# thilinarmtb/lsbench

Hardware: AMD Instinct MI355X
Metric: cg_solves_per_sec (higher is better)
Workload: dtype f64

## Files before the change

include/lsbench_hip.h:

```cpp
#ifndef LSBENCH_HIP_H
#define LSBENCH_HIP_H

#include "lsbench.h"
#include <stddef.h>

#ifdef __cplusplus
extern "C" {
#endif


struct lsbench {
  char *matrix;
  lsbench_solver_t solver;
  lsbench_ordering_t ordering;
  lsbench_precision_t precision;
  unsigned verbose, trials;
};

struct csr {
  unsigned nrows, base;
  unsigned *offs, *cols;
  double *vals;
};

// ... 247 lines not shown
void lsb_plan_exchange(int me, int nall, const unsigned *hull,
                       struct lsb_xfer *recv, int *nrecv,
                       struct lsb_xfer *send, int *nsend);
struct csr *lsbench_matrix_synth(const char *spec, unsigned r0, unsigned r1,
                                 unsigned *n_global);


typedef struct lsb_hip_solver lsb_hip_solver;

lsb_hip_solver *lsb_hip_solver_create(const struct csr *A,
                                      const struct lsb_hip_opts *o);
lsb_hip_solver *lsb_hip_solver_create_dist(const struct csr *A_rows,
                                           unsigned row_begin,
                                           unsigned n_global,
                                           const struct lsb_hip_opts *o);
void lsb_hip_solver_destroy(lsb_hip_solver *s);

int lsb_hip_solver_solve(lsb_hip_solver *s, const double *b, double *x,
                         struct lsb_hip_result *res);
int lsb_hip_solver_solve_dev(lsb_hip_solver *s, const double *d_b, double *d_x,
                             struct lsb_hip_result *res);
int lsb_hip_solver_spmv_dev(lsb_hip_solver *s, const double *d_x, double *d_y);
int lsb_hip_solver_spmv_inner_dev(lsb_hip_solver *s, const double *d_x, double *d_y, double *d_dot);
int lsb_hip_solver_precond_dev(lsb_hip_solver *s, const double *d_r, double *d_z);
int lsb_hip_solver_amg_info(lsb_hip_solver *s, unsigned *levels, unsigned *tail_levels);
int lsb_hip_solver_cheb_interval(const lsb_hip_solver *s, double *lmin, double *lmax);
int lsb_hip_solver_time_spmv(lsb_hip_solver *s, int warm, int reps,
                             double *ms_avg);
int lsb_hip_solver_jacobi_sweep_dev(lsb_hip_solver *s, double w,
                                    const double *d_b, double *d_x);

unsigned lsb_hip_solver_nrows_local(const lsb_hip_solver *s);
int lsb_hip_solver_padded(const lsb_hip_solver *s);
unsigned lsb_hip_solver_nrows_global(const lsb_hip_solver *s);
unsigned long long lsb_hip_solver_nnz_local(const lsb_hip_solver *s);
unsigned lsb_hip_solver_nblocks(const lsb_hip_solver *s);
int lsb_hip_solver_spmv_variant(const lsb_hip_solver *s);
unsigned lsb_hip_solver_spmv_flags(const lsb_hip_solver *s);
unsigned lsb_hip_solver_spmv_grid(const lsb_hip_solver *s);
unsigned lsb_hip_solver_spmv_period(const lsb_hip_solver *s);
unsigned long long lsb_hip_solver_spmv_col_slices(const lsb_hip_solver *s);
void lsb_hip_solver_sell_value_slots(const lsb_hip_solver *s, unsigned *kept, unsigned *total);
int lsb_hip_solver_overlaps(const lsb_hip_solver *s);
int lsb_hip_solver_comm(const lsb_hip_solver *s, double *p2p_us, double *rccl_us);
void lsb_hip_solver_comm_plan(const lsb_hip_solver *s, unsigned long long plan[8]);
int lsb_hip_solver_overlap(const lsb_hip_solver *s, double us[2]);
unsigned long long lsb_hip_solver_spmv_layout_bytes(const lsb_hip_solver *s);
unsigned long long lsb_hip_solver_iteration_bytes(const lsb_hip_solver *s);
int lsb_hip_solver_single_reduction(const lsb_hip_solver *s);
int lsb_hip_solver_fused_p(const lsb_hip_solver *s);
int lsb_hip_solver_blas1_nt(const lsb_hip_solver *s);
void *lsb_hip_stream(void);


#define LSB_HIP_UNIQUE_ID_BYTES 128
int lsb_hip_comm_get_unique_id(void *id128);
int lsb_hip_comm_init_rank(const void *id128, int nranks, int rank);
int lsb_hip_comm_destroy(void);
int lsb_hip_comm_rank(void);
int lsb_hip_comm_size(void);
int lsb_hip_comm_count(void);
int lsb_hip_comm_allreduce_sum_dev(double *d_buf, int count);
int lsb_hip_comm_barrier(void);


#define LSB_SPMV_FLAG_PREFETCH 1u
// ... 36 lines not shown
```

lsbench_amd/_lib.py:

```python
import ctypes as C
import os
import subprocess

_CSRC = os.path.join(os.path.dirname(os.path.abspath(__file__)), "csrc")
LIB_PATH = os.path.join(_CSRC, "liblsbench_hip.so")
CORE_PATH = os.path.join(_CSRC, "liblsbench_core.so")
CORE_SYMBOLS = ("lsbench_matrix_read", "lsbench_matrix_print", "lsbench_matrix_free", "lsbench_init",
                "lsbench_get_matrix_name", "lsbench_bench", "lsbench_finalize")

UNIQUE_ID_BYTES = 128

SOLVER_HIP = 6
OP_CHOLMOD_UPPER, OP_RAW = 0, 1
PRECOND_JACOBI, PRECOND_NONE, PRECOND_L1JACOBI, PRECOND_CHEBYSHEV, PRECOND_BLOCKJACOBI, PRECOND_FSAI = 0, 1, 2, 3, 4, 5
PRECOND_AMG = 6
KRYLOV_PCG, KRYLOV_GMRES, KRYLOV_PCG1, KRYLOV_AUTO, KRYLOV_BICGSTAB = 0, 1, 2, 3, 4
SPMV_AUTO, SPMV_ADAPTIVE, SPMV_SUBWAVE, SPMV_SCALAR, SPMV_PANEL, SPMV_SELL, SPMV_BINNED, SPMV_TWOPHASE = 0, 1, 2, 3, 4, 5, 6, 7
SELL_ROWS = 128
BIN_CHUNK = 2048
PB_COLS, PB_ROWS = 8192, 2048
SPMV_FLAG_PREFETCH, SPMV_FLAG_NT, SPMV_FLAG_C16, SPMV_FLAG_TMPL, SPMV_FLAG_DEFER, SPMV_FLAG_COL = 1, 2, 4, 64, 128, 256
STATUS_RUNNING, STATUS_CONVERGED, STATUS_BREAKDOWN, STATUS_MAXIT = 0, 1, 2, 3
STATUS_COMM = 4
COMM_AUTO, COMM_RCCL, COMM_P2P = 0, 1, 2
# ... 157 lines not shown
    "lsb_sell_vc_free": (None, [C.POINTER(SellVc)]),
    "lsb_csr_fsai_pattern": (C.POINTER(FsaiPattern), [_csrp, _i, _u]),
    "lsb_fsai_pattern_free": (None, [C.POINTER(FsaiPattern)]),
    "lsb_amg_setup": (C.POINTER(AmgHier), [_csrp, _d, _u, _u]),
    "lsb_amg_aggregate": (C.POINTER(C.c_int), [_csrp, _d, C.POINTER(_u)]),
    "lsb_amg_free": (None, [C.POINTER(AmgHier)]),
    "lsb_sell16_templates": (C.POINTER(SellTmpls), [C.POINTER(Sell), C.POINTER(SellVc)]),
    "lsb_sell_tmpls_free": (None, [C.POINTER(SellTmpls)]),
    "lsb_tmpl_check": (_i, [C.POINTER(Sell), C.POINTER(SellVc), C.POINTER(SellTmpls), _u, _u, _u, _i,
                            C.c_char_p, C.c_size_t]),
    "lsb_sell_tmpl_columns": (C.POINTER(TmplCols), [C.POINTER(SellTmpls), _u, _u]),
    "lsb_sell_tmpl_columns_range": (C.POINTER(TmplCols), [C.POINTER(SellTmpls), _u, _u, _u, _u]),
    "lsb_tmpl_cols_free": (None, [C.POINTER(TmplCols)]),
    "lsb_tmpl_cols_check": (_i, [C.POINTER(SellTmpls), C.POINTER(TmplCols), C.c_char_p, C.c_size_t]),
    "lsb_csr_mean_scatter": (_d, [_csrp, _u]),
    "lsb_csr_col_hull": (None, [_csrp, C.POINTER(_u), C.POINTER(_u)]),
    "lsb_plan_exchange": (None, [_i, _i, C.POINTER(_u), C.POINTER(Xfer), C.POINTER(_i),
                                 C.POINTER(Xfer), C.POINTER(_i)]),
    "lsbench_matrix_synth": (_csrp, [C.c_char_p, _u, _u, C.POINTER(_u)]),
    "lsb_hip_solver_create": (_vp, [_csrp, C.POINTER(Opts)]),
    "lsb_hip_solver_create_dist": (_vp, [_csrp, _u, _u, C.POINTER(Opts)]),
    "lsb_hip_solver_destroy": (None, [_vp]),
    "lsb_hip_solver_solve": (_i, [_vp, _vp, _vp, C.POINTER(Result)]),
    "lsb_hip_solver_solve_dev": (_i, [_vp, _vp, _vp, C.POINTER(Result)]),
    "lsb_hip_solver_spmv_dev": (_i, [_vp, _vp, _vp]),
    "lsb_hip_solver_spmv_inner_dev": (_i, [_vp, _vp, _vp, _vp]),
    "lsb_hip_solver_precond_dev": (_i, [_vp, _vp, _vp]),
    "lsb_hip_solver_amg_info": (_i, [_vp, C.POINTER(_u), C.POINTER(_u)]),
    "lsb_hip_solver_cheb_interval": (_i, [_vp, C.POINTER(_d), C.POINTER(_d)]),
    "lsb_hip_solver_time_spmv": (_i, [_vp, _i, _i, C.POINTER(_d)]),
    "lsb_hip_solver_jacobi_sweep_dev": (_i, [_vp, _d, _vp, _vp]),
    "lsb_hip_solver_nrows_local": (_u, [_vp]),
    "lsb_hip_solver_padded": (_i, [_vp]),
    "lsb_csr_pad_lines": (_csrp, [_csrp, _u, C.POINTER(_u), C.POINTER(_u), C.POINTER(C.POINTER(C.c_int))]),
    "lsb_hip_solver_nrows_global": (_u, [_vp]),
    "lsb_hip_solver_nnz_local": (C.c_ulonglong, [_vp]),
    "lsb_hip_solver_nblocks": (_u, [_vp]),
    "lsb_hip_solver_spmv_variant": (_i, [_vp]),
    "lsb_hip_solver_spmv_flags": (_u, [_vp]),
    "lsb_hip_solver_spmv_grid": (_u, [_vp]),
    "lsb_hip_solver_spmv_period": (_u, [_vp]),
    "lsb_hip_solver_spmv_col_slices": (C.c_ulonglong, [_vp]),
    "lsb_hip_solver_sell_value_slots": (None, [_vp, C.POINTER(C.c_uint), C.POINTER(C.c_uint)]),
    "lsb_hip_solver_overlaps": (_i, [_vp]),
    "lsb_hip_solver_overlap": (_i, [_vp, C.POINTER(C.c_double)]),
    "lsb_hip_solver_comm_plan": (None, [_vp, C.POINTER(C.c_ulonglong)]),
    "lsb_hip_solver_spmv_layout_bytes": (C.c_ulonglong, [_vp]),
    "lsb_hip_solver_fused_p": (_i, [_vp]),
    "lsb_hip_solver_iteration_bytes": (C.c_ulonglong, [_vp]),
    "lsb_hip_solver_single_reduction": (_i, [_vp]),
    "lsb_hip_solver_blas1_nt": (_i, [_vp]),
    "lsb_hip_solver_comm": (_i, [_vp, C.POINTER(C.c_double), C.POINTER(C.c_double)]),
    "lsb_hip_stream": (_vp, []),
    "lsb_hip_comm_get_unique_id": (_i, [_vp]),
    "lsb_hip_comm_init_rank": (_i, [_vp, _i, _i]),
    "lsb_hip_comm_destroy": (_i, []),
    "lsb_hip_comm_rank": (_i, []),
    "lsb_hip_comm_size": (_i, []),
    "lsb_hip_comm_count": (_i, []),
    "hip_cdna4_set_option": (_i, [C.c_char_p, C.c_char_p]),
    "hip_cdna4_matrix_synth": (_csrp, [C.c_char_p]),
    "lsb_hip_comm_allreduce_sum_dev": (_i, [_vp, _i]),
    "lsb_hip_comm_barrier": (_i, []),
    "lsb_hip_spmv_csr_f64": (_i, [_i, _u, _vp, _vp, _vp, _vp, _vp, _u, _u, _u, _vp, _vp,
                                  _vp, _vp, _vp, _vp]),
    "lsb_hip_partials_capacity": (_u, []),
# ... 62 lines not shown
```

lsbench_amd/api.py:

```python
import ctypes as C

import numpy as np

from . import _lib as L


def _ptr(a):
    if a is None:
        return None
    if hasattr(a, "data_ptr"):
        return a.data_ptr()
    if isinstance(a, np.ndarray):
        return a.ctypes.data
    return int(a)


class Matrix:

    def __init__(self, handle):
        if not handle:
            raise L.LsbenchHipError("NULL struct csr")
        self._h = handle

    @classmethod
# ... 252 lines not shown
        return lo.value, hi.value

    def time_spmv(self, warm=5, reps=50):
        ms = C.c_double()
        L.check(L.load().lsb_hip_solver_time_spmv(self._h, warm, reps, C.byref(ms)),
                "time_spmv")
        return ms.value

    def jacobi_sweep_dev(self, w, d_b, d_x):
        L.check(L.load().lsb_hip_solver_jacobi_sweep_dev(self._h, w, _ptr(d_b), _ptr(d_x)),
                "jacobi_sweep_dev")

    @property
    def nblocks(self):
        return L.load().lsb_hip_solver_nblocks(self._h)

    @property
    def spmv_variant(self):
        return L.load().lsb_hip_solver_spmv_variant(self._h)

    @property
    def spmv_flags(self):
        return L.load().lsb_hip_solver_spmv_flags(self._h)

    @property
    def spmv_grid(self):
        return L.load().lsb_hip_solver_spmv_grid(self._h)

    @property
    def padded(self):
        return int(L.load().lsb_hip_solver_padded(self._h))

    @property
    def spmv_col_slices(self):
        return int(L.load().lsb_hip_solver_spmv_col_slices(self._h))

    @property
    def spmv_period(self):
        return L.load().lsb_hip_solver_spmv_period(self._h)

    @property
    def sell_value_slots(self):
        import ctypes as C
        k, t = C.c_uint(0), C.c_uint(0)
        L.load().lsb_hip_solver_sell_value_slots(self._h, C.byref(k), C.byref(t))
        return int(k.value), int(t.value)

    @property
    def spmv_layout_bytes(self):
        return int(L.load().lsb_hip_solver_spmv_layout_bytes(self._h))

    @property
    def iteration_bytes(self):
        return int(L.load().lsb_hip_solver_iteration_bytes(self._h))

    @property
    def single_reduction(self):
        return bool(L.load().lsb_hip_solver_single_reduction(self._h))

    @property
    def fused_p(self):
        return int(L.load().lsb_hip_solver_fused_p(self._h))

    @property
    def blas1_nt(self):
        return int(L.load().lsb_hip_solver_blas1_nt(self._h))
# ... 34 lines not shown
```

lsbench_amd/csrc/hip_kernels.hip:

```cpp
#include "hip_kcommon.h"

__device__ __forceinline__ void spmv_publish(double *__restrict__ partials, double dot,
                                             double *sred, const lsb_ar_tail &tail) {
  if (!partials)
    return;
  double d[1] = {dot};
  wg_sum<1>(d, sred);
  if (tail.counter)
    ar_tail(partials, d[0], tail);
  else if (threadIdx.x == 0)
    partials[blockIdx.x] = d[0];
}

enum { SP_PREFETCH = 1, SP_NT = 2 };

template <int FLAGS, class T>
__device__ __forceinline__ T stream_load(const T *p) {
  if (FLAGS & SP_NT)
    return __builtin_nontemporal_load(p);
  return *p;
}

#define LSB_ISSUE_BLOCK(kk)                                                    \
  do {                                                                         \
// ... 1189 lines not shown
        colp_compute<NF, true, XUPD>(c0, m0, pm, p0, pp, down, C, vm0, vm1, vp0, vp1, beta, alpha, alpha2, dc, lane, res, dot);
        COLP_STORE(res, lrow, false, true);
        pm = p0, p0 = pp, c0 = c1, m0 = m1, m1 = m2;
        gu += D, lrow += Du;
      }
      colp_issue_c<NF, false, NT>(c1, C, r, pold, x, pnew, gu + D, D, n, lane);
      colp_compute<NF, true, XUPD>(c0, m0, pm, p0, pp, down, C, vm0, vm1, vp0, vp1, beta, alpha, alpha2, dc, lane, res, dot);
      COLP_STORE(res, lrow, false, true);
      pm = p0, p0 = pp, c0 = c1, m0 = m1;
      gu += D, lrow += Du;
      colp_compute<NF, false, XUPD>(c0, m0, pm, p0, pp, down, C, vm0, vm1, vp0, vp1, beta, alpha, alpha2, dc, lane, res, dot);
      COLP_STORE(res, lrow, false, false);
    } else {
      for (unsigned k = 0; k < K; k++)
        colp_single(s + k * period, n, lane, sptr, sbase, vals, vconst, r, pold, pnew, x, nullptr, beta, alpha, alpha2,
                    XUPD, dc, dot);
    }
  }
  if (partials) {
    double d[1] = {dot};
    wg_sum<1>(d, sred);
    if (threadIdx.x == 0)
      partials[blockIdx.x] = d[0];
  }
}
#undef COLP_STORE
#undef COLP_ST

template <int NF>
__global__ __launch_bounds__(WG, 5) void k_pcg_col_r(
    const unsigned *__restrict__ plan, unsigned period, unsigned n, const unsigned *__restrict__ sptr,
    const unsigned long long *__restrict__ mask, const lsb_sell_tmpl *__restrict__ td, const int *__restrict__ sbase,
    const double *__restrict__ vals, const double *__restrict__ vconst, const double *__restrict__ p,
    double *__restrict__ r, double dc, lsb_pcg_state *__restrict__ st, int parity, int pbuf, int xtwo,
    const double *__restrict__ pq_parts, unsigned npq, double *__restrict__ partials2) {
  static_assert(NF >= 1 && NF <= 2, "one or two far slots per side");
  __shared__ double sred[8];
  const unsigned tid = threadIdx.x, lane = tid & 63u, wave = tid >> 6;
  const unsigned gx = gridDim.x / NXCD, xcd = blockIdx.x % NXCD, slot = blockIdx.x / NXCD;
  const int stopped = st->status, pad = st->pad;
  const double rz = st->rz[parity];
  const unsigned i0 = plan[xcd], i1 = plan[xcd + 1];
  double pqv[1];
  wg_sum_partials<1>(pq_parts, npq, pqv, sred);
  if (stopped)
    return;
  if (pad) {
    if (blockIdx.x == 0 && threadIdx.x == 0)
      st->status = LSB_STATUS_MAXIT;
    return;
  }
  const double pq = pqv[0];
  if (!(pq != 0.0) || !isfinite(pq)) {
    if (blockIdx.x == 0 && threadIdx.x == 0)
      st->status = LSB_STATUS_BREAKDOWN;
    return;
  }
  const double alpha = rz / pq;
  if (blockIdx.x == 0 && threadIdx.x == 0) {
    st->pq = pq, st->alpha[1] = st->alpha[0], st->alpha[0] = alpha, st->xpend = (xtwo ? 3 : 1) + pbuf;
  }
  const u4v *__restrict__ items = (const u4v *)(plan + LSB_COL_HEAD);
  const unsigned dofs = plan[LSB_TMPL_COL_DOWN];
  const unsigned P = period * LSB_SELL_ROWS;
  double acc[2] = {0.0, 0.0}, nodot = 0.0;
#define COLR_FINISH(A0, A1, RV, LROW)                                                          \
  do {                                                                                         \
    sell_d2v rn_;                                                                              \
    rn_.x = (RV).x - alpha * (A0), rn_.y = (RV).y - alpha * (A1);                              \
    *(sell_d2v *)(r + (LROW) + 2 * lane) = rn_;                                                \
    acc[0] += rn_.x * (dc * rn_.x);                                                            \
    acc[0] += rn_.y * (dc * rn_.y);                                                            \
    acc[1] += rn_.x * rn_.x;                                                                   \
    acc[1] += rn_.y * rn_.y;                                                                   \
  } while (0)
  for (unsigned g = slot; i0 + 4 * g < i1; g += gx) {
    const unsigned it = __builtin_amdgcn_readfirstlane(i0 + 4 * g + wave);
    if (it >= i1)
      continue;
    const u4v rec = items[it];
    const unsigned s = __builtin_amdgcn_readfirstlane(rec.x);
    const unsigned K = __builtin_amdgcn_readfirstlane(rec.y) & ~LSB_TMPL_COL_LOCKSTEP;
    if (K >= 3) {
      const unsigned t = __builtin_amdgcn_readfirstlane(rec.z), mb = __builtin_amdgcn_readfirstlane(rec.w);
      const lsb_sell_tmpl *T = td + t;
      col_tmpl<NF> C;
      C.bc = T->base[NF + 1];
      C.k0 = T->cst[0], C.kc = T->cst[NF + 1], C.kL = T->cst[2 * NF + 2];
#pragma unroll
      for (int k = 0; k < NF - 1; k++) {
        C.bl[k] = T->base[1 + k], C.bh[k] = T->base[NF + 3 + k];
        C.kl[k] = T->cst[1 + k], C.kh[k] = T->cst[NF + 3 + k];
      }
      const int side_k[2] = {T->kidx[NF], T->kidx[NF + 2]}, side_kd[2] = {T->kind[NF], T->kind[NF + 2]};
      const bool down = col_walks_down(plan, dofs, it);
      const unsigned s0 = down ? s + (K - 1) * period : s;
      const long long D = down ? -(long long)P : (long long)P;
      const unsigned Du = (unsigned)D;
      long long gu = (long long)s0 * LSB_SELL_ROWS;
      unsigned lrow = s0 * LSB_SELL_ROWS;
      col_ops<NF> cur, nxt;
      sell_d2u cb = *(const sell_d2u *)(p + (gu + C.bc - D) + 2 * lane);
      sell_d2u c0 = *(const sell_d2u *)(p + (gu + C.bc) + 2 * lane);
      sell_d2u ca, cn;
      col_issue<NF, 2>(cur, ca, C, p, r, gu, lrow, D, n, lane, true);
      unsigned long long mk[2][2] = {{0ull, 0ull}, {0ull, 0ull}};
#pragma unroll
      for (int side = 0; side < 2; side++)
        if (side_k[side] >= 0 && side_kd[side] == 2) {
// ... 411 lines not shown
  if (period < NXCD || !plan)
    errx(EXIT_FAILURE, "lsb_k_spmv_tmpl_col: no column plan (period %u)", period);
  const sell_launch L = sell_prologue("lsb_k_spmv_tmpl_col", true, c, nitem, n, grid_cap, 0, period, partials,
                                      npartials, tail_in);
  const int f32 = (flags & LSB_SP_F32) != 0;
  const int dot = !partials || !xdot ? 0 : (xdot == x + row_begin && centre0) ? 1 : 2;
  static decltype(&k_spmv_tmpl_col<1, 0>) const kern[2][3] = {
      {k_spmv_tmpl_col<1, 0>, k_spmv_tmpl_col<1, 1>, k_spmv_tmpl_col<1, 2>},
      {k_spmv_tmpl_col<2, 0>, k_spmv_tmpl_col<2, 1>, k_spmv_tmpl_col<2, 2>}};
  kern[c->tmpl.nfar - 1][dot]<<<L.g, WG, 0, (hipStream_t)stream>>>(
      plan, L.period, n, row_begin, xlen, c->sptr, c->tmpl.mask, c->tmpl.td, c->sbase, c->vals, f32, c->vconst, x, y,
      xdot, partials, st, L.tail);
}

void lsb_k_pcg_col_px(unsigned grid_cap, unsigned period, const unsigned *plan, unsigned nitem, unsigned n,
                      const struct lsb_sell16_dev *c, const double *r, const double *pold, double *pnew, double *x,
                      int xupd, double dc, double *partials, unsigned *npartials, struct lsb_pcg_state *st, int parity,
                      const double *parts2, unsigned nparts2, void *stream) {
  if (period < NXCD || !plan || pold == pnew)
    errx(EXIT_FAILURE, "lsb_k_pcg_col_px: no column plan (period %u) or one direction buffer", period);
  const unsigned nfar = c->tmpl.nfar;
  const sell_launch L = sell_prologue("lsb_k_pcg_col_px", true, c, nitem, n, grid_cap, LSB_TMPL_COL_GRID(nfar), period,
                                      partials, npartials, NULL);
  static decltype(&k_pcg_col_px<1, 3, false>) const kern[2][2] = {
      {k_pcg_col_px<1, 3, false>, k_pcg_col_px<1, 3, true>},
      {k_pcg_col_px<2, 3, false>, k_pcg_col_px<2, 3, true>}};
  kern[nfar - 1][xupd != 0]<<<L.g, WG, 0, (hipStream_t)stream>>>(
      plan, L.period, n, c->sptr, c->tmpl.mask, c->tmpl.td, c->sbase, c->vals, c->vconst, r, pold, pnew, x, dc,
      partials, st, parity, parts2, nparts2);
}

void lsb_k_pcg_col_r(unsigned grid_cap, unsigned period, const unsigned *plan, unsigned nitem, unsigned n,
                     const struct lsb_sell16_dev *c, const double *p, double *r, double dc, struct lsb_pcg_state *st,
                     int parity, int pbuf, int xtwo, const double *pq_parts, unsigned npq, double *partials2,
                     unsigned *npartials, void *stream) {
  if (period < NXCD || !plan)
    errx(EXIT_FAILURE, "lsb_k_pcg_col_r: no column plan (period %u)", period);
  const sell_launch L = sell_prologue("lsb_k_pcg_col_r", true, c, nitem, n, grid_cap, LSB_TMPL_COL_GRID(1), period,
                                      partials2, npartials, NULL);
  const auto kern = c->tmpl.nfar == 1 ? k_pcg_col_r<1> : k_pcg_col_r<2>;
  kern<<<L.g, WG, 0, (hipStream_t)stream>>>(plan, L.period, n, c->sptr, c->tmpl.mask, c->tmpl.td, c->sbase, c->vals,
                                            c->vconst, p, r, dc, st, parity, pbuf, xtwo, pq_parts, npq, partials2);
}

}
```

lsbench_amd/csrc/hip_pcg.c:

```c
#define _GNU_SOURCE
#include "hip_solver.h"

#define DINV(s) ((s)->dinv_uniform ? NULL : (s)->d_dinv), (s)->dinv_const

enum pcg_form pcg_choose_form(const lsb_hip_solver *sv) {
  const struct shard *s = &sv->sh[0];
  const struct lsb_hip_opts *o = &sv->o;
  if (o->krylov == LSB_KRYLOV_GMRES || o->krylov == LSB_KRYLOV_BICGSTAB)
    return PCG_NONE;
  if (o->precond == LSB_PRECOND_FSAI && !sv->multi && !s->mixed && s->variant == LSB_SPMV_SUBWAVE &&
      s->fs_g.variant == LSB_SPMV_SUBWAVE && s->fs_gt.variant == LSB_SPMV_SUBWAVE && o->sample_spmv <= 0 &&
      o->krylov != LSB_KRYLOV_PCG1 && !getenv("LSBENCH_HIP_NO_FSAI_FUSE"))
    return PCG_FSAI3;
  if (generic_precond(sv))
    return PCG_GENERIC;
  if (o->krylov == LSB_KRYLOV_PCG1 || (o->krylov == LSB_KRYLOV_AUTO && sv->multi))
    return PCG_CG1;
  if (sv->multi || s->mixed || getenv("LSBENCH_HIP_NO_FUSE_P"))
    return PCG_CLASSIC;
  if (s->sell_form == SELL_COL && s->dinv_uniform && s->c16.tmpl.nfar >= 1 && s->c16.tmpl.nfar <= 2 &&
      s->row_begin == 0 && s->n == s->n_glob && o->precond == LSB_PRECOND_JACOBI && !getenv("LSBENCH_HIP_NO_FUSE_PX"))
    return PCG_COL;
  return s->variant == LSB_SPMV_SUBWAVE && o->sample_spmv <= 0 ? PCG_SUBWAVE : PCG_CLASSIC;
}
// ... 153 lines not shown
    sv->pcur = 0;
    spmv_shard(s, buf[0], s->d_q, buf[0], s->d_parts_pq, &s->npq, s->d_st);
  } else {
    lsb_k_spmv_subwave_p(s->n, s->csr.offs, s->csr.cols, s->csr.vals, s->lanes, s->d_r, DINV(s),
                         buf[sv->pcur], buf[sv->pcur ^ 1], s->d_q, s->d_parts_pq, &s->npq, s->d_st,
                         parity ^ 1, s->d_parts2, s->np2, g_stream);
    sv->pcur ^= 1;
  }
  lsb_k_pcg_update_xr(s->n, buf[sv->pcur], s->d_q, DINV(s), d_x, s->d_r, s->d_st, parity,
                      s->d_parts_pq, s->npq, s->d_parts2, &s->np2, sv->nt_mask, g_stream);
  if (pos & 2)
    lsb_k_pcg_update_p(s->n, s->d_r, DINV(s), buf[sv->pcur], buf[0], s->d_st, parity, s->d_parts2,
                       s->np2, sv->nt_mask, g_stream);
}

static void col_enqueue_iter(lsb_hip_solver *sv, double *d_x, int parity, int pos, int sample) {
  struct shard *s = &sv->sh[0];
  double *buf[2] = {s->d_pfull, s->d_p1};
  if (sample >= 0)
    sv->samp_skip[sample] = (pos & 1) != 0;
  if (pos & 1) {
    sv->pcur = 0;
    spmv_shard(s, buf[0], s->d_q, buf[0], s->d_parts_pq, &s->npq, s->d_st);
  } else {
    sample_open(sv, sample);
    lsb_k_pcg_col_px(s->sp_grid, s->col.period, s->col.plan, s->col.items, s->n, &s->c16, s->d_r, buf[sv->pcur],
                     buf[sv->pcur ^ 1], d_x,  parity == 0,
                     s->dinv_const, s->d_parts_pq, &s->npq, s->d_st, parity ^ 1, s->d_parts2, s->np2, g_stream);
    sample_close(sv, sample);
    sv->pcur ^= 1;
  }
  lsb_k_pcg_col_r(s->sp_grid, s->col.period, s->col.plan, s->col.items, s->n, &s->c16, buf[sv->pcur], s->d_r,
                  s->dinv_const, s->d_st,
                  parity, sv->pcur,  parity != 0, s->d_parts_pq, s->npq,
                  s->d_parts2, &s->np2, g_stream);
  if (pos & 2) {
    lsb_k_pcg_xfix(s->n, buf[0], buf[1], d_x, s->d_st, g_stream);
    lsb_k_pcg_update_p(s->n, s->d_r, DINV(s), buf[sv->pcur], buf[0], s->d_st, parity, s->d_parts2, s->np2,
                       sv->nt_mask, g_stream);
  }
}

static void cg1_enqueue_init(lsb_hip_solver *sv, const double *d_b, double *d_x) {
  sv->ar_fold = can_fold_allreduce(sv), sv->ar_pending = 0, sv->fold_next = 0;
  for (int i = 0; i < sv->nshard; i++) {
    struct shard *s = &sv->sh[i];
    const size_t o = s->row_begin - sv->row_first, bytes = (size_t)s->n * sizeof(double);
    if (sv->cg1_implicit)
      lsb_k_pcg_init(s->n, d_b + o, DINV(s), d_x + o, s->d_pfull + s->row_begin, s->d_r,
                     s->d_parts2, &s->np2, g_stream);
    else
      lsb_k_pcg_init(s->n, d_b + o, DINV(s), d_x + o, s->d_r, s->d_pfull + s->row_begin,
                     s->d_parts2, &s->np2, g_stream);
    LSB_CHK_HIP(hipMemsetAsync(s->d_p1, 0, bytes, g_stream));
    LSB_CHK_HIP(hipMemsetAsync(s->d_s1, 0, bytes, g_stream));
  }
  init_state(sv);
  spmv_pq(sv, -1);
}

static void cg1_enqueue_iter(lsb_hip_solver *sv, double *d_x, int parity, int sample) {
  for (int i = 0; i < sv->nshard; i++) {
    struct shard *s = &sv->sh[i];
    const size_t o = s->row_begin - sv->row_first;
    double *gr_in = s->d_parts2 + (size_t)parity * 2 * LSB_MAX_PARTIALS;
    double *gr_out = s->d_parts2 + (size_t)(parity ^ 1) * 2 * LSB_MAX_PARTIALS;
    unsigned np2 = 0;
    struct lsb_ar_collect col;
// ... 591 lines not shown
```

lsbench_amd/csrc/hip_solver.c:

```c
#define _GNU_SOURCE
#include "hip_solver.h"
#define NXCD_HOST 8u

unsigned pow2_ceil(unsigned v) {
  unsigned p = 1;
  while (p < v)
    p <<= 1;
  return p;
}

void choose_spmv(struct shard *s, const struct lsb_hip_opts *o) {
  const unsigned mean = s->n ? (unsigned)((s->nnz + s->n - 1) / s->n) : 1;
  int v = o->spmv_variant;
  if (v == LSB_SPMV_AUTO)
    v = s->nnz <= 500000ull ? LSB_SPMV_SUBWAVE : LSB_SPMV_ADAPTIVE;
  if (v == LSB_SPMV_PANEL && !s->panel.n)
    v = LSB_SPMV_ADAPTIVE;
  if (v == LSB_SPMV_BINNED && !s->bins.n)
    v = LSB_SPMV_ADAPTIVE;
  if (v == LSB_SPMV_TWOPHASE && !s->tp.bins)
    v = LSB_SPMV_ADAPTIVE;
  if (v == LSB_SPMV_SELL && !s->sell.sptr)
    v = LSB_SPMV_ADAPTIVE;
  s->variant = v;
// ... 381 lines not shown
  }
  if (s->nnz == 0)
    lo = hi = row_begin;
  s->col_lo = lo, s->col_hi = hi;
  if ((unsigned long long)s->nnz > 0x7FFFFFFFull || n_glob > 0x7FFFFFFFu)
    errx(EXIT_FAILURE, "shard too large for int32 device indices");
  s->mixed = o->precision == LSB_PREC_MIXED, s->exact32 = 1;
  struct csr G = {n, 0, (unsigned *)offs, (unsigned *)cols, (double *)(S->vals + j0)};
  csr_build(s, &G);
  const char *e = getenv("LSBENCH_HIP_PANEL_COLS");
  const unsigned width = e ? (unsigned)strtoul(e, NULL, 10) : 524288u;
  const int scattered = s->nnz > 4000000ull && (double)(hi - lo) * 8.0 > 16.0e6 &&
                        lsb_csr_mean_scatter(&G, row_begin) > 1.0e6;
  if (width && o->spmv_variant == LSB_SPMV_PANEL)
    panel_build(&s->panel, &G, width);
  if (width && (o->spmv_variant == LSB_SPMV_BINNED || (o->spmv_variant == LSB_SPMV_AUTO && scattered)))
    bins_build(&s->bins, &G, width);
  if (o->spmv_variant == LSB_SPMV_TWOPHASE || (o->spmv_variant == LSB_SPMV_AUTO && scattered))
    tp_build(&s->tp, &G, n_glob);
  sell_build(s, &G, o);
  if (s->sell.sptr) {
    struct lsb_sell_vc *V = NULL;
    struct lsb_sell *H = c16_build(s, &G, &V);
    struct lsb_sell_tmpls *TT = V ? tmpl_build(s, H, V) : NULL;
    if (TT)
      col_build(s, H, V, TT);
    LSB_CHK_HIP(hipStreamSynchronize(g_stream));
    lsb_sell_tmpls_free(TT), lsb_sell_vc_free(V), lsb_sell_free(H);
  }
  precond_shard_blocks(s, offs, cols, S->vals + j0, o);
  LSB_CHK_HIP(hipStreamSynchronize(g_stream));
  free(offs), free(cols);

  {
    size_t cnt = 3 * (size_t)n + n_glob;
    if (n_glob > n || o->nvirt > 1 || o->krylov == LSB_KRYLOV_PCG1)
      cnt += 2 * (size_t)n;
    if (o->precond == LSB_PRECOND_CHEBYSHEV)
      cnt += 2 * (size_t)n_glob + (size_t)n;
    else if (o->precond == LSB_PRECOND_BLOCKJACOBI)
      cnt += (size_t)n;
    else if (o->precond == LSB_PRECOND_FSAI)
      cnt += 4 * (size_t)n;
    else if (o->precond == LSB_PRECOND_AMG)
      cnt += 3 * (size_t)n;
    if (o->krylov == LSB_KRYLOV_BICGSTAB)
      cnt += 3 * (size_t)n + n_glob;
    if (o->krylov != LSB_KRYLOV_GMRES && !getenv("LSBENCH_HIP_NO_SLAB") && (size_t)n * sizeof(double) <= ((size_t)160 << 20)) {
      s->slab_cap = cnt * sizeof(double) + 16 * 256;
      if (hipMalloc((void **)&s->d_slab, s->slab_cap) != hipSuccess)
        s->d_slab = NULL, s->slab_cap = 0, (void)hipGetLastError();
    }
  }
  s->d_r = shard_vec(s, n);
  s->d_q = shard_vec(s, n);
  s->d_pfull = shard_vec(s, n_glob);
  s->d_dinv = shard_vec(s, n);
  LSB_CHK_HIP(hipMemsetAsync(s->d_pfull, 0, (size_t)n_glob * sizeof(double), g_stream));
  s->d_parts_pq = (double *)lsb_hip_malloc(3 * LSB_MAX_PARTIALS * sizeof(double));
  s->d_parts2 = (double *)lsb_hip_malloc(4 * LSB_MAX_PARTIALS * sizeof(double));
  s->d_st = (struct lsb_pcg_state *)lsb_hip_malloc(sizeof(struct lsb_pcg_state));
  LSB_CHK_HIP(hipMemsetAsync(s->d_st, 0, sizeof(struct lsb_pcg_state), g_stream));
  s->d_st_aux = (struct lsb_pcg_state *)lsb_hip_malloc(sizeof(struct lsb_pcg_state));
  LSB_CHK_HIP(hipMemsetAsync(s->d_st_aux, 0, sizeof(struct lsb_pcg_state), g_stream));
  choose_spmv(s, o);

  if (o->precond == LSB_PRECOND_JACOBI || o->precond == LSB_PRECOND_L1JACOBI ||
      o->precond == LSB_PRECOND_CHEBYSHEV) {
    int *d_nz = (int *)lsb_hip_malloc(sizeof(int)), nz = 0;
    LSB_CHK_HIP(hipMemsetAsync(d_nz, 0, sizeof(int), g_stream));
    if (o->precond == LSB_PRECOND_L1JACOBI)
      lsb_k_l1_setup(n, s->csr.offs, s->csr.vals, s->d_dinv, d_nz, g_stream);
    else
      lsb_k_jacobi_setup(n, row_begin, s->csr.offs, s->csr.cols, s->csr.vals, s->d_dinv, d_nz,
                         g_stream);
    LSB_CHK_HIP(hipMemcpyAsync(&nz, d_nz, sizeof(int), hipMemcpyDeviceToHost, g_stream));
    LSB_CHK_HIP(hipStreamSynchronize(g_stream));
    lsb_hip_free(d_nz);
    if (nz)
      errx(EXIT_FAILURE, "hip_cdna4: %d rows have no non-zero %s; "
                         "Jacobi preconditioning needs one (cf. the stored-diagonal "
                         "assumption of src/cholmod-impl.h:13)", nz,
           o->precond == LSB_PRECOND_L1JACOBI ? "entry" : "diagonal entry");
  } else {
    double *ones = (double *)malloc((size_t)(n ? n : 1) * sizeof(double));
    for (unsigned i = 0; i < n; i++)
      ones[i] = 1.0;
    LSB_CHK_HIP(hipMemcpy(s->d_dinv, ones, (size_t)n * sizeof(double), hipMemcpyHostToDevice));
    free(ones);
  }
  if (n && !getenv("LSBENCH_HIP_NO_UNIFORM_DINV")) {
// ... 105 lines not shown
  bicgstab_check_precond(&o);
  if (o.precision == LSB_PREC_MIXED && o.precond == LSB_PRECOND_AMG) {
    warnx("hip_cdna4: --precond amg runs in fp64");
    o.precision = LSB_PREC_FP64;
  }
  struct csr *S = o.op_mode == LSB_OP_CHOLMOD_UPPER ? lsb_csr_symmetrize_upper(A)
                                                    : lsb_csr_copy_base0(A);
  const unsigned n_user = S->nrows;
  int *padmap = NULL;
  {
    const char *e = getenv("LSBENCH_HIP_PAD_LINES");
    const int want = e ? atoi(e) : (S->nrows >= 1000000u ? 1 : 0);
    if (want && !o.reorder) {
      unsigned nx = 0, nxp = 0;
      struct csr *Sp = lsb_csr_pad_lines(S, LSB_SELL_ROWS, &nx, &nxp, &padmap);
      if (Sp) {
        if (o.verbose)
          fprintf(stderr, "hip_cdna4: grid lines of %u rows padded to %u (%u -> %u rows)\n", nx, nxp, S->nrows,
                  Sp->nrows);
        lsb_csr_free(S);
        S = Sp;
      }
    }
  }
  int P = o.nvirt > 1 ? o.nvirt : 1;
  if ((unsigned)P > S->nrows / 2)
    P = 1;
  lsb_hip_solver *sv = solver_alloc(P, &o);
  sv->n_user = n_user;
  if (padmap) {
    sv->d_perm = (int *)dev_upload(padmap, (size_t)S->nrows * sizeof(int));
    LSB_CHK_HIP(hipStreamSynchronize(g_stream));
    free(padmap);
    sv->d_bp = (double *)lsb_hip_malloc((size_t)S->nrows * sizeof(double));
    sv->d_xp = (double *)lsb_hip_malloc((size_t)S->nrows * sizeof(double));
    sv->padded = 1;
  }
  if (o.reorder) {
    unsigned *perm = (unsigned *)malloc((size_t)S->nrows * sizeof(unsigned));
    if (!perm || lsb_csr_rcm(S, perm))
      errx(EXIT_FAILURE, "hip_cdna4: out of memory computing the RCM ordering");
    struct csr *Sp = lsb_csr_permute_sym(S, perm);
    if (o.verbose)
      fprintf(stderr, "hip_cdna4: RCM bandwidth %u -> %u\n", lsb_csr_bandwidth(S),
              lsb_csr_bandwidth(Sp));
    lsb_csr_free(S);
    S = Sp;
    sv->d_perm = (int *)dev_upload(perm, (size_t)S->nrows * sizeof(int));
    LSB_CHK_HIP(hipStreamSynchronize(g_stream));
    free(perm);
    sv->d_bp = (double *)lsb_hip_malloc((size_t)S->nrows * sizeof(double));
    sv->d_xp = (double *)lsb_hip_malloc((size_t)S->nrows * sizeof(double));
  }
  sv->n_glob = sv->n_here = S->nrows, sv->row_first = 0;
  sv->dist = 0, sv->multi = P > 1;
  unsigned *bounds = lsb_calloc(unsigned, (size_t)P + 1);
  lsb_csr_partition_rows(S, (unsigned)P, bounds);
  unsigned *hull = lsb_calloc(unsigned, 4 * (size_t)P);
  for (int q = 0; q < P; q++) {
    shard_upload(&sv->sh[q], S, bounds[q], bounds[q + 1], 0, bounds[q], S->nrows, &o);
    hull[4 * q] = bounds[q], hull[4 * q + 1] = bounds[q + 1] - bounds[q];
    hull[4 * q + 2] = sv->sh[q].col_lo, hull[4 * q + 3] = sv->sh[q].col_hi;
  }
  for (int q = 0; q < P; q++) {
    plan_exchange(&sv->sh[q], q, P, hull);
    for (int k = 0; k < sv->sh[q].nrecv; k++)
      if (sv->sh[q].recv[k].count > sv->agree_halo)
        sv->agree_halo = (unsigned)sv->sh[q].recv[k].count;
  }
  free(hull), free(bounds);
  lsb_csr_free(S);
  solver_finish_setup(sv);
  return sv;
}

lsb_hip_solver *lsb_hip_solver_create_dist(const struct csr *A_rows,
                                           unsigned row_begin,
                                           unsigned n_global,
                                           const struct lsb_hip_opts *o_in) {
  if (!lsb_initialized || !A_rows)
    return NULL;
  struct lsb_hip_opts o;
  if (o_in)
    o = *o_in;
  else
    lsb_hip_get_opts(&o);
  if (o.precision == LSB_PREC_MIXED &&
      (o.krylov == LSB_KRYLOV_GMRES || o.krylov == LSB_KRYLOV_BICGSTAB || o.precond == LSB_PRECOND_AMG))
    o.precision = LSB_PREC_FP64;
  bicgstab_check_precond(&o);
  const int P = lsb_hip_comm_size(), me = lsb_hip_comm_rank();
  lsb_hip_solver *sv = solver_alloc(1, &o);
  sv->n_glob = n_global, sv->n_here = sv->n_user = A_rows->nrows, sv->row_first = row_begin;
  const char *alone = getenv("LSBENCH_HIP_DIST_ALONE");
  sv->dist = sv->multi = P > 1 || (alone && atoi(alone) > 0);
// ... 30 lines not shown
    sv->sh[0].nsend = 1, sv->sh[0].send[0].peer = -1;
    sv->sh[0].send[0].offset = row_begin, sv->sh[0].send[0].count = A_rows->nrows;
    sv->sh[0].nrecv = 0;
  }
  free(hull);
  {
    unsigned h = 0, *allh = lsb_calloc(unsigned, (size_t)P);
    for (int k = 0; k < sv->sh[0].nrecv; k++)
      if (sv->sh[0].recv[k].count > h)
        h = (unsigned)sv->sh[0].recv[k].count;
    lsb_hip_comm_allgather_u32(&h, 1, allh);
    for (int q = 0; q < P; q++)
      if (allh[q] > sv->agree_halo)
        sv->agree_halo = allh[q];
    free(allh);
  }
  solver_finish_setup(sv);
  return sv;
}

void lsb_hip_solver_destroy(lsb_hip_solver *sv) {
  if (!sv)
    return;
  LSB_CHK_HIP(hipStreamSynchronize(g_stream));
  drop_graphs(sv);
  if (sv->p2p) {
    if (sv->dist)
      lsb_hip_comm_barrier();
    for (int i = 0; i < sv->nshard; i++)
      lsb_p2p_destroy(sv->p2p[i]);
    free(sv->p2p);
  }
  bicgstab_free(sv);
  for (int i = 0; i < sv->nshard; i++)
    shard_free(&sv->sh[i]);
  if (sv->have_events) {
    for (int i = 0; i < 4 * MAX_SAMPLES; i++)
      LSB_CHK_HIP(hipEventDestroy(sv->ev[i]));
    LSB_CHK_HIP(hipEventDestroy(sv->ev_t0));
    LSB_CHK_HIP(hipEventDestroy(sv->ev_t1));
    LSB_CHK_HIP(hipEventDestroy(sv->ev_poll[0]));
    LSB_CHK_HIP(hipEventDestroy(sv->ev_poll[1]));
    LSB_CHK_HIP(hipEventDestroy(sv->ev_vec));
    LSB_CHK_HIP(hipEventDestroy(sv->ev_halo));
  }
  lsb_hip_free(sv->d_scal_all), lsb_hip_free(sv->d_tmp);
  lsb_hip_free(sv->d_vr), lsb_hip_free(sv->d_ve);
  lsb_hip_free(sv->ps.d_wgrow), lsb_hip_free(sv->ps.d_ug), lsb_hip_free(sv->ps.d_shared);
  lsb_hip_free(sv->d_perm), lsb_hip_free(sv->d_bp), lsb_hip_free(sv->d_xp);
  for (int i = 0; sv->gm && i < sv->nshard; i++) {
    lsb_hip_free(sv->gm[i].V), lsb_hip_free(sv->gm[i].parts);
    lsb_hip_free(sv->gm[i].ax), lsb_hip_free(sv->gm[i].st);
  }
  free(sv->gm);
  lsb_hip_free(sv->gm_red);
  if (sv->gm_hst)
    LSB_CHK_HIP(hipHostFree(sv->gm_hst));
  LSB_CHK_HIP(hipHostFree(sv->h_st));
  free(sv->sh), free(sv);
}

unsigned lsb_hip_solver_nrows_local(const lsb_hip_solver *s) { return s->n_user; }
int lsb_hip_solver_padded(const lsb_hip_solver *s) { return s->padded ? (int)(s->n_here - s->n_user) : 0; }
unsigned lsb_hip_solver_nrows_global(const lsb_hip_solver *s) { return s->n_glob; }
unsigned long long lsb_hip_solver_nnz_local(const lsb_hip_solver *s) {
  unsigned long long z = 0;
  for (int i = 0; i < s->nshard; i++)
    z += s->sh[i].nnz;
  return z;
}
unsigned lsb_hip_solver_nblocks(const lsb_hip_solver *s) { return s->sh[0].csr.nblk; }
int lsb_hip_solver_spmv_variant(const lsb_hip_solver *s) { return s->sh[0].variant; }
unsigned lsb_hip_solver_spmv_flags(const lsb_hip_solver *s) { return s->sh[0].sp_flags; }
unsigned lsb_hip_solver_spmv_grid(const lsb_hip_solver *s) { return s->sh[0].sp_grid; }
unsigned lsb_hip_solver_spmv_period(const lsb_hip_solver *s) { return s->sh[0].sp_period; }
unsigned long long lsb_hip_solver_spmv_col_slices(const lsb_hip_solver *s) { return s->sh[0].col.slices; }
void lsb_hip_solver_sell_value_slots(const lsb_hip_solver *s, unsigned *kept, unsigned *total) {
  const struct shard *h = &s->sh[0];
  const int on = h->sell_form >= SELL_16;
  if (kept)
    *kept = on ? h->c16.vslots : 0;
  if (total)
    *total = on ? h->c16.slots : 0;
}
void lsb_hip_solver_comm_plan(const lsb_hip_solver *s, unsigned long long plan[8]) {
  const struct shard *h = &s->sh[0];
  memset(plan, 0, 8 * sizeof plan[0]);
  plan[0] = (unsigned long long)lsb_hip_comm_count();
  plan[6] = (unsigned long long)s->nshard;
  if (!s->multi)
    return;
  plan[5] = h->nsend == 1 && h->send[0].peer == -1;
  if (plan[5]) {
    const unsigned long long P = s->dist ? (unsigned long long)lsb_hip_comm_size() : (unsigned long long)s->nshard;
    plan[1] = plan[2] = P - 1;
// ... 383 lines not shown
```

lsbench_amd/csrc/hip_solver.h:

```cpp
#ifndef HIP_SOLVER_H
#define HIP_SOLVER_H

#define __HIP_PLATFORM_AMD__ 1
#include <hip/hip_runtime_api.h>
#include <math.h>
#include <string.h>
#include <strings.h>
#include <time.h>

#include "lsb_impl.h"

#define LSB_INTERNAL __attribute__((visibility("hidden")))

extern LSB_INTERNAL int lsb_initialized;
extern LSB_INTERNAL __thread hipStream_t g_stream;
extern LSB_INTERNAL __thread struct lsb_hip_result g_last;
LSB_INTERNAL hipStream_t comm_stream(void);
LSB_INTERNAL void rank_thread_attach(int device);
LSB_INTERNAL void rank_thread_detach(void);
LSB_INTERNAL int bench_multi(double *x, struct csr *A, const double *r, const struct lsbench *cb,
                             const struct lsb_hip_opts *o, int ngpus);

#define SCAL_STRIDE 8
#define MAX_SAMPLES 64
#define LSB_NGRAPH 4

struct halo_split {
  unsigned first, last;
  int ok;
};
enum { SELL_NONE, SELL_32, SELL_16, SELL_TMPL, SELL_COL };
enum pcg_form {
  PCG_NONE,
  PCG_CLASSIC,
  PCG_SUBWAVE,
  PCG_COL,
  PCG_CG1,
  PCG_GENERIC,
  PCG_FSAI3,
};

struct shard {
  char *d_slab;
  size_t slab_cap, slab_used;
  unsigned row_begin, n;
  unsigned long long nnz;
  unsigned n_glob;
  unsigned col_lo, col_hi;
  int variant, sell_form;
  unsigned lanes;
  unsigned sp_flags, sp_grid, sp_period;
  int mixed, exact32;
  struct shard_csr {
    int *offs, *cols, *rowblk;
    unsigned char *blklanes;
    double *vals;
    float *vals32;
    unsigned nblk;
    struct halo_split split;
  } csr;
  struct shard_panel {
    unsigned n;
    unsigned *blk;
    int *offs, *cols, *rowmap, *rowblk;
    unsigned char *blklanes;
    double *vals;
  } panel;
  struct shard_bins {
    unsigned n, cap;
    unsigned *chunk_h;
    unsigned *chunk, *rows, *cols;
    double *vals;
  } bins;
  struct shard_tp {
    unsigned items, bins, col_lo, xlen, cols, rows;
    unsigned *item, *binptr, *first, *delta;
    unsigned long long *mask;
// ... 197 lines not shown
```

lsbench_amd/csrc/lsb_impl.h:

```cpp
#ifndef LSB_IMPL_H
#define LSB_IMPL_H

#include "lsbench_hip.h"
#include <err.h>
#include <stdint.h>
#include <stdio.h>
#include <stdlib.h>

#ifdef __cplusplus
extern "C" {
#endif

#define lsb_calloc(T, n) ((T *)calloc((size_t)(n) > 0 ? (size_t)(n) : 1, sizeof(T)))

struct lsb_pcg_state {
  double rz[2];
  double bb;
  double thresh2;
  double rr;
  double pq;
  double alpha[2];
  int iters;
  int status;
  int maxit;
// ... 66 lines not shown
                     const int *sbase, const double *vals, const double *vconst, unsigned ulen,
                     const double *x, double *y, const double *xdot, double *partials,
                     unsigned *npartials,
                     const struct lsb_pcg_state *st, const struct lsb_ar_tail *tail,
                     const struct lsb_cheb_epi *epi, void *stream);
#define LSB_SP_TMPL 64u
#define LSB_SP_DEFER 128u
struct lsb_sell16_dev {
  unsigned *sptr;
  short *codes;
  int *sbase;
  double *vals;
  double *vconst;
  unsigned vslots, slots, ulen;
  unsigned long long bytes;
  struct lsb_tmpl_dev {
    unsigned *srec;
    unsigned long long *mask;
    struct lsb_sell_tmpl *td;
    unsigned nfar;
    unsigned long long bytes;
  } tmpl;
};
void lsb_k_spmv_tmpl(unsigned flags, unsigned grid_cap, unsigned period, const struct lsb_sell16_dev *c, unsigned s0,
                     unsigned ns, unsigned n, unsigned row_begin, unsigned xlen, const double *x, double *y,
                     const double *xdot, double *partials, unsigned *npartials, const struct lsb_pcg_state *st,
                     const struct lsb_ar_tail *tail, const struct lsb_cheb_epi *epi, void *stream);
void lsb_k_pcg_col_px(unsigned grid_cap, unsigned period, const unsigned *plan, unsigned nitem, unsigned n,
                      const struct lsb_sell16_dev *c, const double *r, const double *pold, double *pnew, double *x,
                      int xupd, double dc, double *partials, unsigned *npartials, struct lsb_pcg_state *st, int parity,
                      const double *parts2, unsigned nparts2, void *stream);
void lsb_k_pcg_col_r(unsigned grid_cap, unsigned period, const unsigned *plan, unsigned nitem, unsigned n,
                     const struct lsb_sell16_dev *c, const double *p, double *r, double dc, struct lsb_pcg_state *st,
                     int parity, int pbuf, int xtwo, const double *pq_parts, unsigned npq, double *partials2,
                     unsigned *npartials, void *stream);
void lsb_k_pcg_xfix(unsigned n, const double *p0, const double *p1, double *x, const struct lsb_pcg_state *st,
                    void *stream);
#define LSB_SP_COL 256u
void lsb_k_spmv_tmpl_col(unsigned flags, unsigned grid_cap, unsigned period, const unsigned *plan, unsigned nitem,
                         int centre0, unsigned n, unsigned row_begin, unsigned xlen, const struct lsb_sell16_dev *c,
                         const double *x, double *y, const double *xdot, double *partials, unsigned *npartials,
                         const struct lsb_pcg_state *st, const struct lsb_ar_tail *tail, void *stream);
void lsb_k_spmv_binned(unsigned flags, unsigned chunk_cap, const unsigned *chunk_begin, unsigned c0,
                       unsigned nchunk, const unsigned *rows, const unsigned *cols, const double *vals,
                       const double *x, double *y, const struct lsb_pcg_state *st, void *stream);
void lsb_k_spmv_twophase(unsigned nitems, const unsigned *item, const double *vals,
                         const unsigned short *colw, const unsigned *grp_first,
                         const unsigned long long *grp_mask, const unsigned *delta,
                         const unsigned short *roww, unsigned col_lo, unsigned cols, unsigned rows,
                         unsigned nbins, const unsigned *bin_ptr, double *prod, unsigned n,
                         const double *x, unsigned xlen, double *y, const double *xdot,
                         double *partials, unsigned *npartials, double *binparts,
                         const struct lsb_pcg_state *st, void *stream);
unsigned lsb_k_twophase_groups(unsigned nbins);
void lsb_k_reduce_final(const double *partials, unsigned nparts, unsigned width,
                        double *out, int take_sqrt,
                        const struct lsb_pcg_state *st, void *stream);
void lsb_k_reduce_final2(const double *pa, unsigned na, unsigned wa, double *outa,
                         const double *pb, unsigned nb, unsigned wb, double *outb,
                         const struct lsb_pcg_state *st, void *stream);
void lsb_k_dot(unsigned n, const double *a, const double *b, double *partials,
               unsigned *npartials, void *stream);
void lsb_k_axpy(unsigned n, const double *alpha, const double *x, double *y,
                void *stream);
void lsb_k_xpay(unsigned n, const double *beta, const double *x, double *y,
                void *stream);
void lsb_k_jacobi_setup(unsigned n, unsigned row_begin, const int *offs,
// ... 183 lines not shown
```

Baseline: 1.099.

## Reverse column-r sweep order and pack p1, permuted b/x vectors into device slab

The fused r-update kernel gains a flag to walk its 4-wave groups in reverse order, and the PCG driver always sets it. The intent is to reuse in cache the tail of the data the previous kernel just touched. The shard slab now also holds the second p buffer (fused-p case) and the permuted b/x vectors for single-shard permuted runs, so these hot vectors sit in one contiguous allocation. A slab_mask query is added to report which vectors landed in the slab. The risks are a changed slab size calculation and a reordered allocation sequence that could affect alignment or locality elsewhere.

```diff
diff --git a/include/lsbench_hip.h b/include/lsbench_hip.h
--- a/include/lsbench_hip.h
+++ b/include/lsbench_hip.h
@@ -303,6 +303,7 @@
 
 unsigned lsb_hip_solver_nrows_local(const lsb_hip_solver *s);
 int lsb_hip_solver_padded(const lsb_hip_solver *s);
+unsigned lsb_hip_solver_slab_mask(const lsb_hip_solver *s);
 unsigned lsb_hip_solver_nrows_global(const lsb_hip_solver *s);
 unsigned long long lsb_hip_solver_nnz_local(const lsb_hip_solver *s);
 unsigned lsb_hip_solver_nblocks(const lsb_hip_solver *s);
diff --git a/lsbench_amd/_lib.py b/lsbench_amd/_lib.py
--- a/lsbench_amd/_lib.py
+++ b/lsbench_amd/_lib.py
@@ -213,6 +213,7 @@
     "lsb_hip_solver_jacobi_sweep_dev": (_i, [_vp, _d, _vp, _vp]),
     "lsb_hip_solver_nrows_local": (_u, [_vp]),
     "lsb_hip_solver_padded": (_i, [_vp]),
+    "lsb_hip_solver_slab_mask": (_u, [_vp]),
     "lsb_csr_pad_lines": (_csrp, [_csrp, _u, C.POINTER(_u), C.POINTER(_u), C.POINTER(C.POINTER(C.c_int))]),
     "lsb_hip_solver_nrows_global": (_u, [_vp]),
     "lsb_hip_solver_nnz_local": (C.c_ulonglong, [_vp]),
diff --git a/lsbench_amd/api.py b/lsbench_amd/api.py
--- a/lsbench_amd/api.py
+++ b/lsbench_amd/api.py
@@ -308,6 +308,10 @@
         return int(L.load().lsb_hip_solver_padded(self._h))
 
     @property
+    def slab_mask(self):
+        return int(L.load().lsb_hip_solver_slab_mask(self._h))
+
+    @property
     def spmv_col_slices(self):
         return int(L.load().lsb_hip_solver_spmv_col_slices(self._h))
 
diff --git a/lsbench_amd/csrc/hip_kernels.hip b/lsbench_amd/csrc/hip_kernels.hip
--- a/lsbench_amd/csrc/hip_kernels.hip
+++ b/lsbench_amd/csrc/hip_kernels.hip
@@ -1245,7 +1245,7 @@
     const unsigned *__restrict__ plan, unsigned period, unsigned n, const unsigned *__restrict__ sptr,
     const unsigned long long *__restrict__ mask, const lsb_sell_tmpl *__restrict__ td, const int *__restrict__ sbase,
     const double *__restrict__ vals, const double *__restrict__ vconst, const double *__restrict__ p,
-    double *__restrict__ r, double dc, lsb_pcg_state *__restrict__ st, int parity, int pbuf, int xtwo,
+    double *__restrict__ r, double dc, lsb_pcg_state *__restrict__ st, int parity, int pbuf, int xtwo, int rev,
     const double *__restrict__ pq_parts, unsigned npq, double *__restrict__ partials2) {
   static_assert(NF >= 1 && NF <= 2, "one or two far slots per side");
   __shared__ double sred[8];
@@ -1287,7 +1287,9 @@
     acc[1] += rn_.x * rn_.x;                                                                   \
     acc[1] += rn_.y * rn_.y;                                                                   \
   } while (0)
-  for (unsigned g = slot; i0 + 4 * g < i1; g += gx) {
+  const unsigned G = (i1 - i0 + 3u) / 4u;
+  for (unsigned j = slot; j < G; j += gx) {
+    const unsigned g = rev ? G - 1u - j : j;
     const unsigned it = __builtin_amdgcn_readfirstlane(i0 + 4 * g + wave);
     if (it >= i1)
       continue;
@@ -1765,7 +1767,7 @@
 
 void lsb_k_pcg_col_r(unsigned grid_cap, unsigned period, const unsigned *plan, unsigned nitem, unsigned n,
                      const struct lsb_sell16_dev *c, const double *p, double *r, double dc, struct lsb_pcg_state *st,
-                     int parity, int pbuf, int xtwo, const double *pq_parts, unsigned npq, double *partials2,
+                     int parity, int pbuf, int xtwo, int rev, const double *pq_parts, unsigned npq, double *partials2,
                      unsigned *npartials, void *stream) {
   if (period < NXCD || !plan)
     errx(EXIT_FAILURE, "lsb_k_pcg_col_r: no column plan (period %u)", period);
@@ -1773,7 +1775,8 @@
                                       partials2, npartials, NULL);
   const auto kern = c->tmpl.nfar == 1 ? k_pcg_col_r<1> : k_pcg_col_r<2>;
   kern<<<L.g, WG, 0, (hipStream_t)stream>>>(plan, L.period, n, c->sptr, c->tmpl.mask, c->tmpl.td, c->sbase, c->vals,
-                                            c->vconst, p, r, dc, st, parity, pbuf, xtwo, pq_parts, npq, partials2);
-}
-
-}
+                                            c->vconst, p, r, dc, st, parity, pbuf, xtwo, rev != 0, pq_parts, npq,
+                                            partials2);
+}
+
+}
diff --git a/lsbench_amd/csrc/hip_pcg.c b/lsbench_amd/csrc/hip_pcg.c
--- a/lsbench_amd/csrc/hip_pcg.c
+++ b/lsbench_amd/csrc/hip_pcg.c
@@ -209,8 +209,8 @@
   }
   lsb_k_pcg_col_r(s->sp_grid, s->col.period, s->col.plan, s->col.items, s->n, &s->c16, buf[sv->pcur], s->d_r,
                   s->dinv_const, s->d_st,
-                  parity, sv->pcur,  parity != 0, s->d_parts_pq, s->npq,
-                  s->d_parts2, &s->np2, g_stream);
+                  parity, sv->pcur,  parity != 0,  1,
+                  s->d_parts_pq, s->npq, s->d_parts2, &s->np2, g_stream);
   if (pos & 2) {
     lsb_k_pcg_xfix(s->n, buf[0], buf[1], d_x, s->d_st, g_stream);
     lsb_k_pcg_update_p(s->n, s->d_r, DINV(s), buf[sv->pcur], buf[0], s->d_st, parity, s->d_parts2, s->np2,
diff --git a/lsbench_amd/csrc/hip_solver.c b/lsbench_amd/csrc/hip_solver.c
--- a/lsbench_amd/csrc/hip_solver.c
+++ b/lsbench_amd/csrc/hip_solver.c
@@ -437,6 +437,8 @@
   LSB_CHK_HIP(hipStreamSynchronize(g_stream));
   free(offs), free(cols);
 
+  const int fused_p = n == n_glob && o->nvirt <= 1 && o->precision == LSB_PREC_FP64 &&
+                      o->precond == LSB_PRECOND_JACOBI && (o->krylov == LSB_KRYLOV_PCG || o->krylov == LSB_KRYLOV_AUTO);
   {
     size_t cnt = 3 * (size_t)n + n_glob;
     if (n_glob > n || o->nvirt > 1 || o->krylov == LSB_KRYLOV_PCG1)
@@ -451,17 +453,25 @@
       cnt += 3 * (size_t)n;
     if (o->krylov == LSB_KRYLOV_BICGSTAB)
       cnt += 3 * (size_t)n + n_glob;
+    if (fused_p)
+      cnt += (size_t)n;
+    if (s->slab_bx)
+      cnt += 2 * (size_t)n;
     if (o->krylov != LSB_KRYLOV_GMRES && !getenv("LSBENCH_HIP_NO_SLAB") && (size_t)n * sizeof(double) <= ((size_t)160 << 20)) {
       s->slab_cap = cnt * sizeof(double) + 16 * 256;
       if (hipMalloc((void **)&s->d_slab, s->slab_cap) != hipSuccess)
         s->d_slab = NULL, s->slab_cap = 0, (void)hipGetLastError();
     }
   }
+  s->d_dinv = shard_vec(s, n);
   s->d_r = shard_vec(s, n);
   s->d_q = shard_vec(s, n);
   s->d_pfull = shard_vec(s, n_glob);
-  s->d_dinv = shard_vec(s, n);
   LSB_CHK_HIP(hipMemsetAsync(s->d_pfull, 0, (size_t)n_glob * sizeof(double), g_stream));
+  if (fused_p) {
+    s->d_p1 = shard_vec(s, n);
+    LSB_CHK_HIP(hipMemsetAsync(s->d_p1, 0, (size_t)n * sizeof(double), g_stream));
+  }
   s->d_parts_pq = (double *)lsb_hip_malloc(3 * LSB_MAX_PARTIALS * sizeof(double));
   s->d_parts2 = (double *)lsb_hip_malloc(4 * LSB_MAX_PARTIALS * sizeof(double));
   s->d_st = (struct lsb_pcg_state *)lsb_hip_malloc(sizeof(struct lsb_pcg_state));
@@ -633,8 +643,6 @@
     sv->d_perm = (int *)dev_upload(padmap, (size_t)S->nrows * sizeof(int));
     LSB_CHK_HIP(hipStreamSynchronize(g_stream));
     free(padmap);
-    sv->d_bp = (double *)lsb_hip_malloc((size_t)S->nrows * sizeof(double));
-    sv->d_xp = (double *)lsb_hip_malloc((size_t)S->nrows * sizeof(double));
     sv->padded = 1;
   }
   if (o.reorder) {
@@ -650,18 +658,24 @@
     sv->d_perm = (int *)dev_upload(perm, (size_t)S->nrows * sizeof(int));
     LSB_CHK_HIP(hipStreamSynchronize(g_stream));
     free(perm);
-    sv->d_bp = (double *)lsb_hip_malloc((size_t)S->nrows * sizeof(double));
-    sv->d_xp = (double *)lsb_hip_malloc((size_t)S->nrows * sizeof(double));
   }
   sv->n_glob = sv->n_here = S->nrows, sv->row_first = 0;
   sv->dist = 0, sv->multi = P > 1;
   unsigned *bounds = lsb_calloc(unsigned, (size_t)P + 1);
   lsb_csr_partition_rows(S, (unsigned)P, bounds);
   unsigned *hull = lsb_calloc(unsigned, 4 * (size_t)P);
+  sv->sh[0].slab_bx = sv->d_perm && P == 1;
   for (int q = 0; q < P; q++) {
     shard_upload(&sv->sh[q], S, bounds[q], bounds[q + 1], 0, bounds[q], S->nrows, &o);
     hull[4 * q] = bounds[q], hull[4 * q + 1] = bounds[q + 1] - bounds[q];
     hull[4 * q + 2] = sv->sh[q].col_lo, hull[4 * q + 3] = sv->sh[q].col_hi;
+  }
+  if (sv->sh[0].slab_bx) {
+    sv->d_xp = shard_vec(&sv->sh[0], S->nrows);
+    sv->d_bp = shard_vec(&sv->sh[0], S->nrows);
+  } else if (sv->d_perm) {
+    sv->d_bp = (double *)lsb_hip_malloc((size_t)S->nrows * sizeof(double));
+    sv->d_xp = (double *)lsb_hip_malloc((size_t)S->nrows * sizeof(double));
   }
   for (int q = 0; q < P; q++) {
     plan_exchange(&sv->sh[q], q, P, hull);
@@ -758,6 +772,7 @@
     free(sv->p2p);
   }
   bicgstab_free(sv);
+  shard_vec_free(&sv->sh[0], sv->d_bp), shard_vec_free(&sv->sh[0], sv->d_xp);
   for (int i = 0; i < sv->nshard; i++)
     shard_free(&sv->sh[i]);
   if (sv->have_events) {
@@ -773,7 +788,7 @@
   lsb_hip_free(sv->d_scal_all), lsb_hip_free(sv->d_tmp);
   lsb_hip_free(sv->d_vr), lsb_hip_free(sv->d_ve);
   lsb_hip_free(sv->ps.d_wgrow), lsb_hip_free(sv->ps.d_ug), lsb_hip_free(sv->ps.d_shared);
-  lsb_hip_free(sv->d_perm), lsb_hip_free(sv->d_bp), lsb_hip_free(sv->d_xp);
+  lsb_hip_free(sv->d_perm);
   for (int i = 0; sv->gm && i < sv->nshard; i++) {
     lsb_hip_free(sv->gm[i].V), lsb_hip_free(sv->gm[i].parts);
     lsb_hip_free(sv->gm[i].ax), lsb_hip_free(sv->gm[i].st);
@@ -787,6 +802,15 @@
 }
 
 unsigned lsb_hip_solver_nrows_local(const lsb_hip_solver *s) { return s->n_user; }
+unsigned lsb_hip_solver_slab_mask(const lsb_hip_solver *sv) {
+  const struct shard *s = &sv->sh[0];
+  const void *v[5] = {s->d_r, s->d_pfull, s->d_p1, sv->d_xp, sv->d_bp};
+  unsigned m = 0;
+  for (int k = 0; k < 5; k++)
+    if (v[k] && s->d_slab && (const char *)v[k] >= s->d_slab && (const char *)v[k] < s->d_slab + s->slab_cap)
+      m |= 1u << k;
+  return m;
+}
 int lsb_hip_solver_padded(const lsb_hip_solver *s) { return s->padded ? (int)(s->n_here - s->n_user) : 0; }
 unsigned lsb_hip_solver_nrows_global(const lsb_hip_solver *s) { return s->n_glob; }
 unsigned long long lsb_hip_solver_nnz_local(const lsb_hip_solver *s) {
diff --git a/lsbench_amd/csrc/hip_solver.h b/lsbench_amd/csrc/hip_solver.h
--- a/lsbench_amd/csrc/hip_solver.h
+++ b/lsbench_amd/csrc/hip_solver.h
@@ -43,6 +43,7 @@
 struct shard {
   char *d_slab;
   size_t slab_cap, slab_used;
+  int slab_bx;
   unsigned row_begin, n;
   unsigned long long nnz;
   unsigned n_glob;
diff --git a/lsbench_amd/csrc/lsb_impl.h b/lsbench_amd/csrc/lsb_impl.h
--- a/lsbench_amd/csrc/lsb_impl.h
+++ b/lsbench_amd/csrc/lsb_impl.h
@@ -122,7 +122,7 @@
                       const double *parts2, unsigned nparts2, void *stream);
 void lsb_k_pcg_col_r(unsigned grid_cap, unsigned period, const unsigned *plan, unsigned nitem, unsigned n,
                      const struct lsb_sell16_dev *c, const double *p, double *r, double dc, struct lsb_pcg_state *st,
-                     int parity, int pbuf, int xtwo, const double *pq_parts, unsigned npq, double *partials2,
+                     int parity, int pbuf, int xtwo, int rev, const double *pq_parts, unsigned npq, double *partials2,
                      unsigned *npartials, void *stream);
 void lsb_k_pcg_xfix(unsigned n, const double *p0, const double *p1, double *x, const struct lsb_pcg_state *st,
                     void *stream);
```

New measurement: 1.124 (median of 6 runs). +2.3%, better.
